# FabricioArendTorres/FlowConductor

Hardware: AMD Instinct MI355X
Metric: log_prob samples/sec, 32xRQ-NSF coupling D=64 K=8 (higher is better)
Workload: dtype f32

## Files before the change

flowconductor_amd/csrc/fc_rq_eval_plan.h:

```cpp
#pragma once
#include <hip/hip_runtime.h>
#include <utility>

#ifndef FC_GEN_SHIFT
#define FC_GEN_SHIFT 0
#endif

namespace fc {

template <class F, int... I>
__device__ __forceinline__ void static_for(F&& f, std::integer_sequence<int, I...>) {
  (f(std::integral_constant<int, I>{}), ...);
}

template <int K, int HOOKS, bool kHookReads, bool kBox>
struct EvalPlan {
  enum Section {
    sInside, sBoxErr, sMaxInit, sRead, sDer,
    sMax, sSub, sExp, sSumInit, sSum, sTot, sRcpX, sRcpY, sKnot, sSelect, sBin, sDelta, sTheta,
    sSoftExp, sSoftFix, sSoftLog, sSoftDer,
    sSoftExp1, sSoftFix1, sSoftLog1, sSoftDer1,
    sDsum, sQuadratic, sT1mt, sDn1, sDnum, sLog, sLval, sYs, sOut, kSections
  };
  struct Sec { int count, weight; };
  static constexpr Sec kSecs[kSections] = {
      {1, 3},
      {kBox ? 1 : 0, 1},
      {1, 1},
      {K, 3},
      {kBox ? K + 1 : K - 1, 1},
      {1, 0},
      {K, 1},
      {K, 4},
      {1, 0},
      {K - 2, 1},
      {1, 1},
      {1, 5},
      {1, 6},
      {2 * (K - 1), 2},
      {1, 3}, {1, 2},
      {1, 5}, {1, 4},
      {1, 6}, {1, 3}, {1, 10}, {1, 3},
      {1, 6}, {1, 3}, {1, 10}, {1, 3},
      {1, 3}, {1, 2},
      {1, 4}, {1, 5}, {1, 4},
      {1, 3}, {1, 1},
      {1, 8}, {1, 3},
  };
  static constexpr int first(int section) {
    int c = 0;
    for (int s = 0; s < section; ++s) c += kSecs[s].count;
    return c;
  }
  static constexpr int kChunks = first(kSections);
  static constexpr int weight(int chunk) {
    int s = 0;
    while (chunk >= kSecs[s].count) chunk -= kSecs[s++].count;
    return kSecs[s].weight;
  }
  static constexpr int hooks_until(int chunk) {
    if (chunk == kChunks - 1) return HOOKS;
    const int start = kHookReads ? 0 : first(sMax);
    int total = 0, acc = 0, hook = 0;
    for (int c = start; c < kChunks; ++c) total += weight(c);
    for (int c = start; c <= chunk; ++c) {
      acc += weight(c);
      while (hook < HOOKS && acc * HOOKS * 100 >= ((hook + 1) * 100 - (FC_GEN_SHIFT)) * total) ++hook;
    }
    return hook;
  }
};

}
```

flowconductor_amd/csrc/fc_rq_eval_straight.inc:

```
{
  using std::integral_constant, std::make_integer_sequence;
  auto chunk_end = [&](auto C) {
    constexpr int c = decltype(C)::value, h0 = c > 0 ? Plan::hooks_until(c - 1) : 0, h1 = Plan::hooks_until(c);
    static_for([&](auto J) { hook(integral_constant<int, h0 + decltype(J)::value>{}); }, make_integer_sequence<int, h1 - h0>{});
  };
#define FC_CHUNK_END(section, i) chunk_end(integral_constant<int, Plan::first(Plan::section) + (i)>{})
  constexpr int H = K / 2;

  const bool inside = (x >= q.left) && (x <= q.right);
  const float xc = inside ? x : q.left;
  FC_CHUNK_END(sInside, 0);
  if constexpr (!kTails) {
    if (!inside) err |= kErrOutsideDomain;
    FC_CHUNK_END(sBoxErr, 0);
  }
  float mx = -INFINITY, my = -INFINITY;
  FC_CHUNK_END(sMaxInit, 0);
  FC_F2 t[K];
  static_for([&](auto I) {
    t[I] = FC_F2{FC_WH(I), FC_WH(K + I)};
    mx = fmaxf(mx, t[I].x);
    my = fmaxf(my, t[I].y);
    FC_CHUNK_END(sRead, I);
  }, make_integer_sequence<int, K>{});
  static_for([&](auto J) {
    FC_DER_ST(kTails ? J + 1 : J, FC_UD(J));
    FC_CHUNK_END(sDer, J);
  }, make_integer_sequence<int, kTails ? K - 1 : K + 1>{});
  const FC_F2 m = {mx, my};
  FC_CHUNK_END(sMax, 0);
  static_for([&](auto I) {
    t[I] = t[I] - m;
    FC_CHUNK_END(sSub, I);
  }, make_integer_sequence<int, K>{});
  static_for([&](auto I) {
    t[I] = FC_F2{__builtin_amdgcn_exp2f(t[I].x), __builtin_amdgcn_exp2f(t[I].y)};
    FC_CHUNK_END(sExp, I);
  }, make_integer_sequence<int, K>{});
  FC_F2 l[H], r[K - 1];
  l[0] = t[0];
  r[K - 2] = t[K - 1];
  FC_CHUNK_END(sSumInit, 0);
  static_for([&](auto N) {
    if constexpr (N < H - 1) {
      l[N + 1] = l[N] + t[N + 1];
      FC_CHUNK_END(sSum, 2 * N);
    }
    r[K - 3 - N] = r[K - 2 - N] + t[K - 2 - N];
    FC_CHUNK_END(sSum, N < H - 1 ? 2 * N + 1 : 2 * N);
  }, make_integer_sequence<int, K - H - 1>{});
  const FC_F2 tot = l[H - 1] + r[H - 1];
  FC_CHUNK_END(sTot, 0);
  const float rsx = div_lean(1.f, tot.x);
  FC_CHUNK_END(sRcpX, 0);
  const float rsy = div_lean(1.f, tot.y);
  const FC_F2 gk = sc1 * FC_F2{rsx, rsy};
  int idx = 0;
  FC_CHUNK_END(sRcpY, 0);
  static_for([&](auto I) {
    FC_F2 next;
    if constexpr (I < H) next = __builtin_elementwise_fma(l[I], gk, kc[I]);
    else next = __builtin_elementwise_fma(r[I], -gk, kc[I]);
    FC_KNOT_ST(I + 1, next);
    FC_CHUNK_END(sKnot, 2 * I);
    FC_COUNT_GE(idx, xc, kInv ? next.y : next.x);
    FC_CHUNK_END(sKnot, 2 * I + 1);
  }, make_integer_sequence<int, K - 1>{});
  const int bin = idx;
  const FC_F2 sel_lo = FC_KNOT_LD(bin, 0), sel_hi = FC_KNOT_LD(bin, 1);
  const float u[2] = {FC_DER_LD(bin, 0), FC_DER_LD(bin, 1)};
  FC_CHUNK_END(sSelect, 0);
  const float xk = sel_lo.x, yk = sel_lo.y;
  const float wk = sel_hi.x - sel_lo.x, hk = sel_hi.y - sel_lo.y;
  FC_CHUNK_END(sBin, 0);
  const float rwk = __builtin_amdgcn_rcpf(wk);
  const float dq = hk * rwk;
  const float delta = __builtin_fmaf(__builtin_fmaf(-wk, dq, hk), rwk, dq);
  FC_CHUNK_END(sDelta, 0);
  float theta;
  if constexpr (!kInv) {
    const float tq = (xc - xk) * rwk;
    theta = __builtin_fmaf(__builtin_fmaf(-wk, tq, xc - xk), rwk, tq);
  }
  FC_CHUNK_END(sTheta, 0);
  float d[2];
  static_for([&](auto N) {
    const float xb = u[N];
    const float xm = fminf(xb, 20.f);
    const float ex = __builtin_amdgcn_exp2f(xm * 1.4426950408889634f);
    FC_CHUNK_END(sSoftExp + 4 * N, 0);
    const float up = 1.f + ex;
    const float rr = ex - (up - 1.f);
    FC_CHUNK_END(sSoftFix + 4 * N, 0);
    const float l1p = __builtin_fmaf(__builtin_amdgcn_logf(up), 0.6931471805599453f, rr * __builtin_amdgcn_rcpf(up));
    FC_CHUNK_END(sSoftLog + 4 * N, 0);
    d[N] = q.min_d + (xb > 20.f ? xb : l1p) * inv_beta;
    FC_CHUNK_END(sSoftDer + 4 * N, 0);
  }, make_integer_sequence<int, 2>{});
  const float d0 = d[0], d1 = d[1];
  const float dsum = d0 + d1 - 2.f * delta;
  FC_CHUNK_END(sDsum, 0);
  if constexpr (kInv) {
    const float rr = xc - yk;
    const float qa = rr * dsum + hk * (delta - d0);
    const float qb = hk * d0 - rr * dsum;
    const float qc = -delta * rr;
    const float disc = qb * qb - 4.f * qa * qc;
    if (inside && !(disc >= 0.f)) err |= kErrDiscriminant;
    theta = div_lean(2.f * qc, -qb - sqrt_lean(disc));
  }
  FC_CHUNK_END(sQuadratic, 0);
  const float t1mt = theta * (1.f - theta);
  const float den = delta + dsum * t1mt;
  FC_CHUNK_END(sT1mt, 0);
  const float omt = 1.f - theta;
  const float dn1 = d1 * (theta * theta) + 2.f * delta * t1mt;
  FC_CHUNK_END(sDn1, 0);
  const float dnum = (delta * delta) * (dn1 + d0 * (omt * omt));
  FC_CHUNK_END(sDnum, 0);
  const float l2v = __builtin_fmaf(-2.f, __builtin_amdgcn_logf(den), __builtin_amdgcn_logf(dnum));
  FC_CHUNK_END(sLog, 0);
  const float lval = l2v * 0.6931471805599453f;
  FC_CHUNK_END(sLval, 0);
  float ys;
  if constexpr (!kInv) {
    const float num = hk * (delta * (theta * theta) + d0 * t1mt);
    ys = yk + div_lean(num, den);
  } else {
    ys = theta * wk + xk;
  }
  FC_CHUNK_END(sYs, 0);
  y = inside ? ys : x;
  lad = inside ? (kInv ? -lval : lval) : 0.f;
  FC_CHUNK_END(sOut, 0);
  static_assert(Plan::kSecs[Plan::sBoxErr].count == (kTails ? 0 : 1) && Plan::kSecs[Plan::sRead].count == K &&
                    Plan::kSecs[Plan::sDer].count == (kTails ? K - 1 : K + 1) && Plan::kSecs[Plan::sSub].count == K &&
                    Plan::kSecs[Plan::sExp].count == K && Plan::kSecs[Plan::sSum].count == (H - 1) + (K - H - 1) &&
                    Plan::kSecs[Plan::sKnot].count == 2 * (K - 1),
                "the plan and this fragment count the same chunks");
#undef FC_CHUNK_END
}
```

flowconductor_amd/csrc/fc_rq_fused3.hip:

```cpp
#include <hip/hip_runtime.h>
#include <stdint.h>
#include <type_traits>
#include "fc_tile.h"
#include "fc_math.h"
#include "fc_rq_op.h"
#include "fc_rq_eval_plan.h"
#include "fc_rq_fused.h"
#include "fc_split.h"
#include "fc_lane.h"
#include "../../include/flowcon_hip.h"

#ifndef FC_ABL
#define FC_ABL 0
#endif

namespace fc {

#ifndef FC_HOOK_MASK
#define FC_HOOK_MASK 0
#endif
#define FC_F2 f2
#ifndef FC_PRIO_PERIOD
#define FC_PRIO_PERIOD 36
#endif

constexpr int kCt3 = 6;
constexpr int kHB = kH + 16;
constexpr int kKnotFloats = (kK + 1) * 64 * 2;
constexpr int kDerFloats = (kK + 1) * 64;
constexpr int kTabBytes = 8 * (kKnotFloats + kDerFloats) * 4;

template <int R>
struct Fused3Lds {
  static constexpr int kHPiece = R * kHB;
  static constexpr int kHbufBytes = 2 * 2 * kHPiece * 2;
  static constexpr int kLpartBytes = 3 * 8 * R * 4;
  static constexpr int kHscaleBytes = 3 * R * 4;
  static constexpr size_t bytes(int d) {
    return (size_t)kHbufBytes + kLpartBytes + kHscaleBytes + kTabBytes + 3 * R * (d + 4) * 4 + kDt * 4;
  }
};

size_t fused3_lds_bytes(int d, int rows) { return rows == 64 ? Fused3Lds<64>::bytes(d) : Fused3Lds<32>::bytes(d); }

template <bool kInv, int R, int XV, bool kFull, bool kPadX>
__global__ __launch_bounds__(512) void rq_fused_linear_kernel3(RQOp<kK> op, FusedArgs a) {
  using L = Fused3Lds<R>;
  constexpr int kHPiece = L::kHPiece;
  constexpr int NB = R / 16;
  constexpr int HV = R / 32;
  extern __shared__ __attribute__((aligned(16))) unsigned char smem3[];
  _Float16* hbuf = reinterpret_cast<_Float16*>(smem3);
  float* lpart = reinterpret_cast<float*>(smem3 + L::kHbufBytes);
  float* hscale = lpart + 3 * 8 * R;
  float* tabs = hscale + 3 * R;
  float* xbuf = tabs + kTabBytes / 4;
  const int D = a.D, XS = kPadX ? D + 4 : D;
  int* cs = reinterpret_cast<int*>(xbuf + 3 * R * (D + 4));

  const int tid = threadIdx.x, wave = tid >> 6, lane = tid & 63;
  const int s16 = lane & 15, g = lane >> 4;
  const int64_t stride = gridDim.x;
  const int64_t tile0 = blockIdx.x;
  if (tile0 >= a.tiles) return;
  if (tid < kDt) cs[tid] = tid < a.dt ? a.cols[tid] : 0;
  const int WD = kFull ? 8 : (a.dt + 3) >> 2;
  const bool dim_ok = kFull || 4 * wave + g < a.dt;
  const bool active = kFull || wave < WD;
  const float inv_div = op.inv_div;
#if FC_ABL & 16
  const uint64_t stamp_r_entry = __builtin_amdgcn_s_memrealtime();
#endif

  constexpr auto slot_param = [](int s) { return s < 16 ? ((s & 1) ? 8 + (s >> 1) : (s >> 1)) : s; };
  f16x8 wh[kCt3][2], wl[kCt3][2];
  float w_unscale;
  {
    float wv[kCt3][2][8];
    float wmax = 0.f;
#pragma unroll
    for (int t = 0; t < kCt3; ++t) {
      const int wdim = 4 * (active ? wave : 0) + (s16 >> 2), wprm = slot_param(4 * t + (s16 & 3));
      const bool wreal = wprm < kPP - 1 && wdim < a.dt;
      const int row = wreal ? wdim * a.wrows + wprm : 0;
      const float wmask = wreal ? 1.f : 0.f;
#pragma unroll
      for (int ks = 0; ks < 2; ++ks) {
        const float4* src = reinterpret_cast<const float4*>(a.wpad + (int64_t)row * kH + 32 * ks + 8 * g);
        const float4 v0 = src[0], v1 = src[1];
        const float v[8] = {v0.x * wmask, v0.y * wmask, v0.z * wmask, v0.w * wmask,
                            v1.x * wmask, v1.y * wmask, v1.z * wmask, v1.w * wmask};
#pragma unroll
        for (int j = 0; j < 8; ++j) {
          wv[t][ks][j] = v[j];
          wmax = fmaxf(wmax, fabsf(v[j]));
        }
      }
    }
#pragma unroll
    for (int o = 32; o > 0; o >>= 1) wmax = fmaxf(wmax, __shfl_xor(wmax, o));
    float w_scale;
    pow2_scale(wmax, w_scale, w_unscale);
#pragma unroll
    for (int t = 0; t < kCt3; ++t)
#pragma unroll
      for (int ks = 0; ks < 2; ++ks)
#pragma unroll
        for (int j = 0; j < 8; ++j) {
          _Float16 ph, pl;
          split2(wv[t][ks][j] * w_scale, ph, pl);
          wh[t][ks][j] = ph;
          wl[t][ks][j] = pl;
        }
  }
  const float wh_mul = (float)((double)inv_div * 1.4426950408889634);
  f32x4 bw[kCt3];
#pragma unroll
  for (int t = 0; t < kCt3; ++t) {
    const int bdim = 4 * (active ? wave : 0) + g;
    const float* bsrc = a.bias + bdim * a.wrows;
    const float m = t < 4 ? wh_mul : op.q.beta;
    const bool bdim_ok = bdim < a.dt;
    auto bias_of = [&](int slot) {
      const int prm = slot_param(slot);
      const bool real = prm < kPP - 1 && bdim_ok;
      return (real ? bsrc[prm] : a.bias[0]) * (real ? m : 0.f);
    };
    bw[t] = f32x4{bias_of(4 * t), bias_of(4 * t + 1), bias_of(4 * t + 2), bias_of(4 * t + 3)};
  }
  const double span_x = (double)op.q.right - (double)op.q.left, span_y = (double)op.q.top - (double)op.q.bottom;
  const f2 sc1 = {(float)(span_x * (double)op.q.cw), (float)(span_y * (double)op.q.ch)};
  auto knot_const = [&](int i) {
    if (i < kK / 2)
      return f2{(float)((double)op.q.left + span_x * (double)op.q.min_w * (double)(i + 1)),
                (float)((double)op.q.bottom + span_y * (double)op.q.min_h * (double)(i + 1))};
    return f2{(float)((double)op.q.right - span_x * (double)op.q.min_w * (double)(kK - 1 - i)),
              (float)((double)op.q.top - span_y * (double)op.q.min_h * (double)(kK - 1 - i))};
  };
  f2 kc[kK - 1];
  static_for([&](auto I) { kc[I] = knot_const(I); }, std::make_integer_sequence<int, kK - 1>{});

  float* ktab = tabs + wave * (kKnotFloats + kDerFloats) + lane * 2;
  float* dtab = tabs + wave * (kKnotFloats + kDerFloats) + kKnotFloats + lane;
  *reinterpret_cast<f2*>(ktab) = f2{op.q.left, op.q.bottom};
  *reinterpret_cast<f2*>(ktab + kK * 128) = f2{op.q.right, op.q.top};
  dtab[0] = op.q.tail_const * op.q.beta;
  dtab[kK * 64] = op.q.tail_const * op.q.beta;

  uint32_t err = 0;
  int mycol = 0;
  const int xvec = R * D / 4;
  constexpr bool kCarry = kFull && XV <= 2;
  float4 hv0, hv1, xv0, xv1, xv2, xv3;
  hv0 = hv1 = xv0 = xv1 = xv2 = xv3 = float4{0.f, 0.f, 0.f, 0.f};
  int64_t fetched = tile0;
  auto fetch = [&](int64_t t) __attribute__((always_inline)) {
    fetched = t;
    if (FC_ABL & 8) t = tile0;
    const float4* hg = reinterpret_cast<const float4*>(a.h + t * R * kH);
    hv0 = hg[tid];
    if constexpr (HV > 1 && kFull) hv1 = hg[tid + 512];
    const float4* xg = reinterpret_cast<const float4*>(a.x + t * R * D);
    xv0 = xg[tid < xvec ? tid : 0];
    if constexpr (kCarry) {
      if constexpr (XV > 1) xv1 = xg[tid + 512 < xvec ? tid + 512 : 0];
      if constexpr (XV > 2) xv2 = xg[tid + 1024 < xvec ? tid + 1024 : 0];
      if constexpr (XV > 3) xv3 = xg[tid + 1536 < xvec ? tid + 1536 : 0];
    }
  };
  auto xslot = [&](int buf, int i) __attribute__((always_inline)) {
    if constexpr (!kPadX) return reinterpret_cast<float4*>(xbuf + buf * R * XS + 4 * i);
    const int e = i * 4, r = e / D, c = e - r * D;
    return reinterpret_cast<float4*>(xbuf + (buf * R + r) * XS + c);
  };
  auto park_h = [&](int buf, int xbuf3, int k, const float4& hvk) __attribute__((always_inline)) {
    const int c = (tid & 15) * 4, r = (tid >> 4) + 32 * k;
#if FC_ABL & 32
    {
      _Float16* dst = hbuf + (buf * 2 * R + r) * kHB + c;
      *reinterpret_cast<u32x2*>(dst) = u32x2{__float_as_uint(hvk.x) & 0x3bff3bffu, __float_as_uint(hvk.y) & 0x3bff3bffu};
      *reinterpret_cast<u32x2*>(dst + kHPiece) = u32x2{__float_as_uint(hvk.z) & 0x3bff3bffu, __float_as_uint(hvk.w) & 0x3bff3bffu};
      if ((tid & 15) == 0) hscale[xbuf3 * R + r] = 1.f;
      return;
    }
#endif
    const float v[4] = {hvk.x, hvk.y, hvk.z, hvk.w};
    const float m = row16_allmax(fmaxf(fmaxf(fabsf(v[0]), fabsf(v[1])), fmaxf(fabsf(v[2]), fabsf(v[3]))));
    float sc, un;
    pow2_scale(m, sc, un);
    u32x2 p0, p1;
#pragma unroll
    for (int j = 0; j < 2; ++j) {
      uint32_t ph, pl;
      split2_pair(v[2 * j], v[2 * j + 1], sc, ph, pl);
      p0[j] = ph; p1[j] = pl;
    }
    _Float16* dst = hbuf + (buf * 2 * R + r) * kHB + c;
    *reinterpret_cast<u32x2*>(dst) = p0;
    *reinterpret_cast<u32x2*>(dst + kHPiece) = p1;
    if ((tid & 15) == 0) hscale[xbuf3 * R + r] = un;
  };
  auto park = [&](int hb2, int x3) __attribute__((always_inline)) {
    park_h(hb2, x3, 0, hv0);
    if constexpr (HV > 1 && !kFull)
      hv1 = reinterpret_cast<const float4*>(a.h + ((FC_ABL & 8) ? tile0 : fetched) * R * kH)[tid + 512];
    if constexpr (HV > 1) park_h(hb2, x3, 1, hv1);
    if (tid < xvec) *xslot(x3, tid) = xv0;
    if constexpr (!kCarry && XV > 1) {
      const float4* xg = reinterpret_cast<const float4*>(a.x + ((FC_ABL & 8) ? tile0 : fetched) * R * D);
      xv1 = xg[tid + 512 < xvec ? tid + 512 : 0];
      if constexpr (XV > 2) xv2 = xg[tid + 1024 < xvec ? tid + 1024 : 0];
      if constexpr (XV > 3) xv3 = xg[tid + 1536 < xvec ? tid + 1536 : 0];
    }
    if constexpr (XV > 1) if (tid + 512 < xvec) *xslot(x3, tid + 512) = xv1;
    if constexpr (XV > 2) if (tid + 1024 < xvec) *xslot(x3, tid + 1024) = xv2;
    if constexpr (XV > 3) if (tid + 1536 < xvec) *xslot(x3, tid + 1536) = xv3;
  };
  auto hfrag = [&](int hb, int blk, int hp, int ks) {
    return *reinterpret_cast<const f16x8*>(hbuf + ((hb * 2 + hp) * R + 16 * blk + s16) * kHB + 32 * ks + 8 * g);
  };

  auto mfma_n = [&](auto N, f32x4 (&acc)[kCt3], const f16x8& bcur) {
    constexpr int n = decltype(N)::value, term = n / 12, ks = (n / 6) % 2, t = n % 6;
    const f16x8& aop = term == 0 ? wl[t][ks] : wh[t][ks];
    acc[t] = __builtin_amdgcn_mfma_f32_16x16x32_f16(aop, bcur, n < kCt3 ? f32x4{0.f, 0.f, 0.f, 0.f} : acc[t], 0, 0, 0);
  };
  constexpr auto term_h = [](int term) { return term == 1 ? 1 : 0; };

#define FC_ALL36(M)                                                                                          \
  M(0) M(1) M(2) M(3) M(4) M(5) M(6) M(7) M(8) M(9) M(10) M(11) M(12) M(13) M(14) M(15) M(16) M(17) M(18)     \
  M(19) M(20) M(21) M(22) M(23) M(24) M(25) M(26) M(27) M(28) M(29) M(30) M(31) M(32) M(33) M(34) M(35)

  auto produce_only = [&](f32x4 (&acc)[kCt3], int hb, int blk) {
    f16x8 bcur = hfrag(hb, blk, term_h(0), 0);
    auto one = [&](auto N) {
      constexpr int n = decltype(N)::value;
      if constexpr (n % 6 == 0 && n > 0) bcur = hfrag(hb, blk, term_h(n / 12), (n / 6) % 2);
      mfma_n(N, acc, bcur);
    };
#define FC_S(n) one(std::integral_constant<int, n>{});
    FC_ALL36(FC_S)
#undef FC_S
  };

  auto step = [&](const f32x4 (&pa)[kCt3], int xb, int cblk, f32x4 (&acc)[kCt3], int hb, int pblk, float& lad_out) {
    float* xr = xbuf + (xb * R + 16 * cblk + s16) * XS + mycol;
    const float x = *xr;
    const float c_d = hscale[xb * R + 16 * cblk + s16] * w_unscale;
    const float c_wh = c_d * wh_mul;
    const float c_ud = c_d * op.q.beta;
    f16x8 bcur, bnext = hfrag(hb, pblk, term_h(0), 0);
    auto hook = [&](auto N) {
      constexpr int n = decltype(N)::value;
      if constexpr (n % 6 == 0) {
        bcur = bnext;
        if constexpr (n + 6 < 36) bnext = hfrag(hb, pblk, term_h((n + 6) / 12), ((n + 6) / 6) % 2);
      }
      if constexpr (!(FC_ABL & 4)) mfma_n(N, acc, bcur);
      if constexpr (n % (FC_PRIO_PERIOD / 4) == FC_PRIO_PERIOD / 4 - 1)
        __builtin_amdgcn_s_setprio(3 - ((n + 1) % FC_PRIO_PERIOD) / (FC_PRIO_PERIOD / 4));
      __builtin_amdgcn_sched_barrier(FC_HOOK_MASK);
    };
    constexpr int K = kK;
    constexpr bool kTails = true;
    using Plan = EvalPlan<kK, 6 * kCt3, true, false>;
    const RQParams& q = op.q;
    const float inv_beta = op.inv_beta;
    float y, lad;
    __builtin_amdgcn_s_setprio(3);
    __builtin_amdgcn_sched_barrier(0);
#define FC_HOOK(n) hook(std::integral_constant<int, n>{});
#define FC_WH_SLOT(i) ((i) < 8 ? 2 * (i) : 2 * ((i) - 8) + 1)
#define FC_WH(i) __builtin_fmaf(pa[FC_WH_SLOT(i) >> 2][FC_WH_SLOT(i) & 3], c_wh, bw[FC_WH_SLOT(i) >> 2][FC_WH_SLOT(i) & 3])
#define FC_UD(j) __builtin_fmaf(pa[((j) + 16) >> 2][((j) + 16) & 3], c_ud, bw[((j) + 16) >> 2][((j) + 16) & 3])
#define FC_KNOT_ST(slot, v) *reinterpret_cast<f2*>(ktab + (slot) * 128) = (v)
#define FC_KNOT_LD(i, off) *reinterpret_cast<const f2*>(ktab + ((i) + (off)) * 128)
#define FC_DER_ST(slot, v) dtab[(slot) * 64] = (v)
#define FC_DER_LD(i, off) dtab[((i) + (off)) * 64]
#define FC_COUNT_GE(count, a, b)                                                              \
  do {                                                                                        \
    const float fc_b_ = (b);                                                                  \
    asm("v_cmp_ge_f32 vcc, %1, %2\n\tv_addc_co_u32 %0, vcc, 0, %0, vcc" : "+v"(count) : "v"(a), "v"(fc_b_) : "vcc"); \
  } while (0)
#if FC_ABL & 1
    FC_ALL36(FC_HOOK)
    y = x + (FC_WH(0) + FC_WH(5) + FC_WH(10) + FC_WH(15) + FC_UD(0) + FC_UD(5)) * 0.f + q.left * 0.f;
    lad = 0.f;
#else
#include "fc_rq_eval_straight.inc"
#endif
#undef FC_COUNT_GE
#undef FC_DER_LD
#undef FC_DER_ST
#undef FC_KNOT_LD
#undef FC_KNOT_ST
#undef FC_UD
#undef FC_WH
#undef FC_WH_SLOT
#undef FC_HOOK
    if (dim_ok) *xr = y;
    lad_out = dim_ok ? lad : 0.f;
  };
  auto after_steps = [&](int xb, const float (&lb)[NB]) __attribute__((always_inline)) {
    if constexpr (NB == 4) {
      const float l = lane_merge16(lb[0], lane_merge32(lb[2], lb[3]));
      lpart[(xb * 8 + wave) * R + 16 * rows4_sum4_index(g) + s16] = l;
    } else {
      const float m = lane_merge32(lb[0], lb[1]);
      const float l = m + lane_xor16(m, lane);
      if ((g & 1) == 0) lpart[(xb * 8 + wave) * R + 16 * (g >> 1) + s16] = l;
    }
  };

#if FC_ABL & 16
  const uint64_t stamp_c0 = __builtin_amdgcn_s_memtime(), stamp_r0 = __builtin_amdgcn_s_memrealtime();
#endif
#if FC_ABL & 16
  uint64_t barrier_wait = 0, phase_cyc[6] = {0, 0, 0, 0, 0, 0}, phase_t = __builtin_amdgcn_s_memtime();
#define FC_PHASE(k)                                              \
  do {                                                           \
    const uint64_t now = __builtin_amdgcn_s_memtime();           \
    phase_cyc[k] += now - phase_t;                               \
    phase_t = now;                                               \
  } while (0)
#define FC_TIMED_BARRIER()                                        \
  do {                                                            \
    const uint64_t b0 = __builtin_amdgcn_s_memtime();             \
    __syncthreads();                                              \
    barrier_wait += __builtin_amdgcn_s_memtime() - b0;            \
  } while (0)
#else
#define FC_TIMED_BARRIER() __syncthreads()
#define FC_PHASE(k)
#endif
  f32x4 acc0[kCt3], acc1[kCt3];
#pragma unroll
  for (int t = 0; t < kCt3; ++t) acc0[t] = acc1[t] = f32x4{0.f, 0.f, 0.f, 0.f};
  auto write_out = [&](int64_t t, int x3) __attribute__((always_inline)) {
    float4* yg = reinterpret_cast<float4*>(a.y + t * R * D);
#pragma unroll
    for (int k = 0; k < XV; ++k)
      if (tid + 512 * k < xvec) yg[tid + 512 * k] = *xslot(x3, tid + 512 * k);
    if (tid < R) {
      const float* lp = lpart + x3 * 8 * R + tid;
      float l = lp[0];
#pragma unroll
      for (int w = 1; w < 8; ++w)
        if (w < WD) l += lp[w * R];
      a.logabsdet[t * R + tid] = a.accumulate ? a.logabsdet[t * R + tid] + l : l;
    }
  };
  fetch(tile0);
  park(0, 0);
  __syncthreads();
  mycol = cs[(4 * wave + g) & (kDt - 1)];
  if (active) produce_only(acc0, 0, 0);
  int hb = 0, x3 = 0;
  int64_t prev_tile = -1;
  for (int64_t tile = tile0; tile < a.tiles; tile += stride) {
    const bool has_next = tile + stride < a.tiles;
    const int x3n = x3 == 2 ? 0 : x3 + 1, x3p = x3 == 0 ? 2 : x3 - 1;
    FC_PHASE(0);
    if (has_next) fetch(tile + stride);
    float lb[NB];
#pragma unroll
    for (int b = 0; b < NB; ++b) lb[b] = 0.f;
    if (active) {
      step(acc0, x3, 0, acc1, hb, 1, lb[0]);
      if constexpr (NB == 4) {
        step(acc1, x3, 1, acc0, hb, 2, lb[1]);
        lb[0] = lane_merge32(lb[0], lb[1]);
        step(acc0, x3, 2, acc1, hb, 3, lb[2]);
      }
    }
    FC_PHASE(1);
    if (has_next) park(hb ^ 1, x3n);
    FC_PHASE(2);
    FC_TIMED_BARRIER();
    FC_PHASE(3);
    if (prev_tile >= 0) write_out(prev_tile, x3p);
    FC_PHASE(5);
    if (active) {
      step(acc1, x3, NB - 1, acc0, hb ^ 1, 0, lb[NB - 1]);
      after_steps(x3, lb);
    }
    FC_PHASE(4);
    prev_tile = tile;
    hb ^= 1;
    x3 = x3n;
  }
  __syncthreads();
  if (prev_tile >= 0) write_out(prev_tile, x3 == 0 ? 2 : x3 - 1);
#if FC_ABL & 16
  if (tid == 0) {
    a.y[tile0 * R * D] = (float)(__builtin_amdgcn_s_memtime() - stamp_c0);
    a.y[tile0 * R * D + 1] = (float)(__builtin_amdgcn_s_memrealtime() - stamp_r0);
    a.y[tile0 * R * D + 2] = (float)(stamp_r0 - stamp_r_entry);
    a.y[tile0 * R * D + 3] = (float)(stamp_r_entry & 0xffffff);
  }
  if (lane == 0) {
    a.y[tile0 * R * D + 4 + wave] = (float)barrier_wait;
#pragma unroll
    for (int k = 0; k < 6; ++k) a.y[tile0 * R * D + 12 + wave * 6 + k] = (float)phase_cyc[k];
  }
#endif
  if (err && a.err) atomicOr(a.err, err);
}
#undef FC_ALL36
#undef FC_TIMED_BARRIER
#undef FC_PHASE

template <bool kInv, int R, int XV, bool kFull, bool kPadX>
static hipError_t launch_cfg(const RQOp<kK>& op, const FusedArgs& a, unsigned grid, hipStream_t stream) {
  const size_t lds = Fused3Lds<R>::bytes(a.D);
  if (lds > 160 * 1024) return hipErrorInvalidConfiguration;
  static PerDeviceOnce attr;
  const hipError_t ea = ensure_max_dynamic_lds(
      attr, reinterpret_cast<const void*>(&rq_fused_linear_kernel3<kInv, R, XV, kFull, kPadX>), 160 * 1024);
  if (ea != hipSuccess) return ea;
  hipLaunchKernelGGL((rq_fused_linear_kernel3<kInv, R, XV, kFull, kPadX>), dim3(grid), dim3(512), lds, stream, op, a);
  return hipGetLastError();
}

template <bool kInv, int R, int XV>
static hipError_t launch_one(const RQOp<kK>& op, const FusedArgs& a, unsigned grid, hipStream_t stream) {
  if (a.D & 3) return launch_cfg<kInv, R, XV, false, false>(op, a, grid, stream);
  return a.dt == kDt ? launch_cfg<kInv, R, XV, true, true>(op, a, grid, stream)
                     : launch_cfg<kInv, R, XV, false, true>(op, a, grid, stream);
}

hipError_t launch_fused3(const RQOp<kK>& op, const FusedArgs& a, int rows, unsigned grid, hipStream_t stream) {
  const bool inv = op.q.inverse != 0;
  if (rows == 64) {
    if (a.D <= 32) return inv ? launch_one<true, 64, 1>(op, a, grid, stream) : launch_one<false, 64, 1>(op, a, grid, stream);
    if (a.D <= 64) return inv ? launch_one<true, 64, 2>(op, a, grid, stream) : launch_one<false, 64, 2>(op, a, grid, stream);
    return inv ? launch_one<true, 64, 4>(op, a, grid, stream) : launch_one<false, 64, 4>(op, a, grid, stream);
  }
  if (a.D <= 64) return inv ? launch_one<true, 32, 1>(op, a, grid, stream) : launch_one<false, 32, 1>(op, a, grid, stream);
  return inv ? launch_one<true, 32, 2>(op, a, grid, stream) : launch_one<false, 32, 2>(op, a, grid, stream);
}

}
```

flowconductor_amd/csrc/fc_rq_fused4_body.h:

```cpp
#include <hip/hip_runtime.h>
#include <stdint.h>
#include <type_traits>
#include <utility>
#include "fc_device.h"
#include "fc_lane.h"
#include "fc_math.h"
#include "fc_rq_eval_plan.h"
#include "fc_rq_fused_general.h"
#include "fc_rq_op.h"
#include "fc_split.h"
#include "fc_tile.h"

#define FC_F4_CAT2(a, b) a##b
#define FC_F4_CAT(a, b) FC_F4_CAT2(a, b)

namespace fc {
namespace FC_F4_CAT(f4, FC_F4_NAME) {

#define FC_F2 f2
constexpr int K = FC_F4_K;
constexpr bool kTails = FC_F4_TAILS != 0;
constexpr int P = kTails ? 3 * K - 1 : 3 * K + 1;
constexpr int CT = (P + 3) / 4;
constexpr int PP = 4 * CT;
constexpr int NM = 6 * CT;
using Plan = EvalPlan<K, NM, false, !kTails>;
constexpr int R = 32;
constexpr int kHB = 64 + 16;
constexpr int kBiasRow = 36;
constexpr int kKnotFloats = (K + 1) * 64 * 2;
constexpr int kDerFloats = (K + 1) * 64;
constexpr int kTabBytes = 8 * (kKnotFloats + kDerFloats) * 4;
constexpr int kHPiece = R * kHB;
constexpr int kHbufBytes = 2 * 2 * kHPiece * 2;
constexpr int kLpartBytes = 3 * 8 * R * 4;
constexpr int kHscaleBytes = 3 * R * 4;
constexpr int kBiasBytes = 8 * 4 * kBiasRow * 4;
static_assert(PP <= 32 && K <= 11 && K >= 4, "accumulator slots / knot constants");

constexpr size_t lds_bytes(int d) {
  return (size_t)kHbufBytes + kLpartBytes + kHscaleBytes + kTabBytes + kBiasBytes + (size_t)3 * R * (d + 4) * 4 + 32 * 4;
}

template <bool kInv, int XV, bool kFull, bool kPadX>
__global__ __launch_bounds__(512) void rq_fused_linear_kernel4(RQOp<K> op, GenArgs a) {
  extern __shared__ __attribute__((aligned(16))) unsigned char smem4[];
  _Float16* hbuf = reinterpret_cast<_Float16*>(smem4);
  float* lpart = reinterpret_cast<float*>(smem4 + kHbufBytes);
  float* hscale = lpart + 3 * 8 * R;
  float* tabs = hscale + 3 * R;
  float* bias_lds = tabs + kTabBytes / 4;
  float* xbuf = bias_lds + 8 * 4 * kBiasRow;
  const int D = a.D, XS = kPadX ? D + 4 : D;
  int* cs = reinterpret_cast<int*>(xbuf + 3 * R * (D + 4));

  const int tid = threadIdx.x, wave = tid >> 6, lane = tid & 63;
  const int s16 = lane & 15, g = lane >> 4;
  const int64_t stride = gridDim.x;
  const int64_t tile0 = blockIdx.x;
  if (tile0 >= a.tiles) return;
  if (tid < 32) cs[tid] = a.cols[tid < a.dt ? tid : 0];
  const int WD = kFull ? 8 : (a.dt + 3) >> 2;
  const bool dim_ok = kFull || 4 * wave + g < a.dt;
  const bool active = kFull || wave < WD;
  const int grp = active ? wave : 0;

  auto slot_param = [](int s) { return s < 2 * K ? ((s & 1) ? K + (s >> 1) : (s >> 1)) : s; };
  f16x8 wh[CT][2], wl[CT][2];
  {
    const f16x8* wbase = a.wfrag + (size_t)grp * 2 * CT * 2 * 64;
#pragma unroll
    for (int t = 0; t < CT; ++t) {
      const int p = slot_param(4 * t + (lane & 3));
      const int st = p >> 2, sl = (lane & ~3) | (p & 3);
#pragma unroll
      for (int ks = 0; ks < 2; ++ks) {
        wh[t][ks] = wbase[((ks * CT + st) * 2 + 0) * 64 + sl];
        wl[t][ks] = wbase[((ks * CT + st) * 2 + 1) * 64 + sl];
      }
    }
  }
  const float w_unscale = a.wun[grp];
  const float inv_div = op.inv_div;
  const float wh_mul = (float)((double)inv_div * 1.4426950408889634);
  for (int i = tid; i < WD * 4 * PP; i += 512) {
    const int row = i / PP, slot = i - row * PP;
    const int prm = slot_param(slot);
    bias_lds[row * kBiasRow + slot] = a.bias[row * PP + prm] * (slot < 2 * K ? wh_mul : op.q.beta);
  }
  const f32x4* bwp = reinterpret_cast<const f32x4*>(bias_lds + (grp * 4 + g) * kBiasRow);

  const RQParams& q = op.q;
  const f2 sc1 = {q.sc1x, q.sc1y};
  f2 kc[K - 1];
  static_for([&](auto I) { kc[I] = f2{q.kcx[I], q.kcy[I]}; }, std::make_integer_sequence<int, K - 1>{});

  float* ktab = tabs + wave * (kKnotFloats + kDerFloats) + lane * 2;
  float* dtab = tabs + wave * (kKnotFloats + kDerFloats) + kKnotFloats + lane;
  *reinterpret_cast<f2*>(ktab) = f2{q.left, q.bottom};
  *reinterpret_cast<f2*>(ktab + K * 128) = f2{q.right, q.top};
  if constexpr (kTails) {
    dtab[0] = q.tail_const * q.beta;
    dtab[K * 64] = q.tail_const * q.beta;
  }

  uint32_t err = 0;
  int mycol = 0;
  const int xvec = R * D / 4;
  float4 hv0, xv0, xv1;
  hv0 = xv0 = xv1 = float4{0.f, 0.f, 0.f, 0.f};
  auto fetch = [&](int64_t t) __attribute__((always_inline)) {
    hv0 = reinterpret_cast<const float4*>(a.h + t * R * 64)[tid];
    const float4* xg = reinterpret_cast<const float4*>(a.x + t * R * D);
    xv0 = xg[tid < xvec ? tid : 0];
    if constexpr (XV > 1) xv1 = xg[tid + 512 < xvec ? tid + 512 : 0];
  };
  auto xslot = [&](int buf, int i) __attribute__((always_inline)) {
    if constexpr (!kPadX) return reinterpret_cast<float4*>(xbuf + buf * R * XS + 4 * i);
    const int e = i * 4, r = e / D, c = e - r * D;
    return reinterpret_cast<float4*>(xbuf + (buf * R + r) * XS + c);
  };
  auto park = [&](int hb2, int x3) __attribute__((always_inline)) {
    const int c = (tid & 15) * 4, r = tid >> 4;
    const float v[4] = {hv0.x, hv0.y, hv0.z, hv0.w};
    const float m = row16_allmax(fmaxf(fmaxf(fabsf(v[0]), fabsf(v[1])), fmaxf(fabsf(v[2]), fabsf(v[3]))));
    float sc, un;
    pow2_scale(m, sc, un);
    u32x2 p0, p1;
#pragma unroll
    for (int j = 0; j < 2; ++j) {
      uint32_t ph, pl;
      split2_pair(v[2 * j], v[2 * j + 1], sc, ph, pl);
      p0[j] = ph; p1[j] = pl;
    }
    _Float16* dst = hbuf + (hb2 * 2 * R + r) * kHB + c;
    *reinterpret_cast<u32x2*>(dst) = p0;
    *reinterpret_cast<u32x2*>(dst + kHPiece) = p1;
    if ((tid & 15) == 0) hscale[x3 * R + r] = un;
    if (tid < xvec) *xslot(x3, tid) = xv0;
    if constexpr (XV > 1) if (tid + 512 < xvec) *xslot(x3, tid + 512) = xv1;
  };
  auto hfrag = [&](int hb, int blk, int hp, int ks) {
    return *reinterpret_cast<const f16x8*>(hbuf + ((hb * 2 + hp) * R + 16 * blk + s16) * kHB + 32 * ks + 8 * g);
  };
  auto mfma_n = [&](auto N, f32x4 (&acc)[CT], const f16x8& bcur) {
    constexpr int n = decltype(N)::value, term = n / (2 * CT), ks = (n / CT) % 2, t = n % CT;
    const f16x8& aop = term == 0 ? wl[t][ks] : wh[t][ks];
    acc[t] = __builtin_amdgcn_mfma_f32_16x16x32_f16(aop, bcur, n < CT ? f32x4{0.f, 0.f, 0.f, 0.f} : acc[t], 0, 0, 0);
  };
  constexpr auto term_h = [](int term) { return term == 1 ? 1 : 0; };

  auto produce_only = [&](f32x4 (&acc)[CT], int hb, int blk) {
    f16x8 bcur = hfrag(hb, blk, term_h(0), 0);
    static_for([&](auto N) {
      constexpr int n = decltype(N)::value;
      if constexpr (n % CT == 0 && n > 0) bcur = hfrag(hb, blk, term_h(n / (2 * CT)), (n / CT) % 2);
      mfma_n(N, acc, bcur);
    }, std::make_integer_sequence<int, NM>{});
  };

  auto step = [&](f32x4 (&acc)[CT], int xb, int cblk, int hb, int pblk, float& lad_out) {
    float* xr = xbuf + (xb * R + 16 * cblk + s16) * XS + mycol;
    const float x = *xr;
    const float c_d = hscale[xb * R + 16 * cblk + s16] * w_unscale;
    const float c_wh = c_d * wh_mul;
    const float c_ud = c_d * q.beta;
    f32x4 bw[CT];
#pragma unroll
    for (int t = 0; t < CT; ++t) bw[t] = bwp[t];
    f16x8 bcur, bnext = hfrag(hb, pblk, term_h(0), 0);
    constexpr int PQ = (NM + 3) / 4;
    auto hook = [&](auto N) {
      constexpr int n = decltype(N)::value;
      if constexpr (n % CT == 0) {
        bcur = bnext;
        if constexpr (n + CT < NM) bnext = hfrag(hb, pblk, term_h((n + CT) / (2 * CT)), ((n + CT) / CT) % 2);
      }
      mfma_n(N, acc, bcur);
      if constexpr (n % PQ == PQ - 1 || n == NM - 1) __builtin_amdgcn_s_setprio(3 - ((n + 1) % NM) / PQ);
      __builtin_amdgcn_sched_barrier(0);
    };
    const float inv_beta = op.inv_beta;
    float y, lad;
    __builtin_amdgcn_s_setprio(3);
    __builtin_amdgcn_sched_barrier(0);
#define FC_WH_SLOT(i) ((i) < K ? 2 * (i) : 2 * ((i) - K) + 1)
#define FC_WH(i) __builtin_fmaf(acc[FC_WH_SLOT(i) >> 2][FC_WH_SLOT(i) & 3], c_wh, bw[FC_WH_SLOT(i) >> 2][FC_WH_SLOT(i) & 3])
#define FC_UD(j) __builtin_fmaf(acc[((j) + 2 * K) >> 2][((j) + 2 * K) & 3], c_ud, bw[((j) + 2 * K) >> 2][((j) + 2 * K) & 3])
#define FC_KNOT_ST(slot, v) *reinterpret_cast<f2*>(ktab + (slot) * 128) = (v)
#define FC_KNOT_LD(i, off) *reinterpret_cast<const f2*>(ktab + ((i) + (off)) * 128)
#define FC_DER_ST(slot, v) dtab[(slot) * 64] = (v)
#define FC_DER_LD(i, off) dtab[((i) + (off)) * 64]
#define FC_COUNT_GE(count, a, b)                                                              \
  do {                                                                                        \
    const float fc_b_ = (b);                                                                  \
    asm("v_cmp_ge_f32 vcc, %1, %2\n\tv_addc_co_u32 %0, vcc, 0, %0, vcc" : "+v"(count) : "v"(a), "v"(fc_b_) : "vcc"); \
  } while (0)
#include "fc_rq_eval_straight.inc"
#undef FC_COUNT_GE
#undef FC_DER_LD
#undef FC_DER_ST
#undef FC_KNOT_LD
#undef FC_KNOT_ST
#undef FC_UD
#undef FC_WH
#undef FC_WH_SLOT
    if (dim_ok) *xr = y;
    lad_out = dim_ok ? lad : 0.f;
  };
  auto after_steps = [&](int xb, float l0, float l1) __attribute__((always_inline)) {
    const float m = lane_merge32(l0, l1);
    const float l = m + lane_xor16(m, lane);
    if ((g & 1) == 0) lpart[(xb * 8 + wave) * R + 16 * (g >> 1) + s16] = l;
  };

  f32x4 acc[CT];
#pragma unroll
  for (int t = 0; t < CT; ++t) acc[t] = f32x4{0.f, 0.f, 0.f, 0.f};
  auto write_out = [&](int64_t t, int x3) __attribute__((always_inline)) {
    float4* yg = reinterpret_cast<float4*>(a.y + t * R * D);
#pragma unroll
    for (int k = 0; k < XV; ++k)
      if (tid + 512 * k < xvec) yg[tid + 512 * k] = *xslot(x3, tid + 512 * k);
    if (tid < R) {
      const float* lp = lpart + x3 * 8 * R + tid;
      float l = lp[0];
#pragma unroll
      for (int w = 1; w < 8; ++w)
        if (w < WD) l += lp[w * R];
      a.logabsdet[t * R + tid] = a.accumulate ? a.logabsdet[t * R + tid] + l : l;
    }
  };
#ifdef FC_F4_STAMP
  const uint64_t stamp_c0 = __builtin_amdgcn_s_memtime(), stamp_r0 = __builtin_amdgcn_s_memrealtime();
  uint64_t phase_cyc[6] = {0, 0, 0, 0, 0, 0}, phase_t = stamp_c0;
#define FC_PHASE(k)                                              \
  do {                                                           \
    const uint64_t now = __builtin_amdgcn_s_memtime();           \
    phase_cyc[k] += now - phase_t;                               \
    phase_t = now;                                               \
  } while (0)
#else
#define FC_PHASE(k)
#endif
  fetch(tile0);
  park(0, 0);
  __syncthreads();
  mycol = cs[(4 * wave + g) & 31];
  if (active) produce_only(acc, 0, 0);
  int hb = 0, x3 = 0;
  int64_t prev_tile = -1;
  for (int64_t tile = tile0; tile < a.tiles; tile += stride) {
    const bool has_next = tile + stride < a.tiles;
    const int x3n = x3 == 2 ? 0 : x3 + 1, x3p = x3 == 0 ? 2 : x3 - 1;
    FC_PHASE(0);
    if (has_next) fetch(tile + stride);
    float lb0 = 0.f, lb1 = 0.f;
    if (active) step(acc, x3, 0, hb, 1, lb0);
    FC_PHASE(1);
    if (has_next) park(hb ^ 1, x3n);
    FC_PHASE(2);
    __syncthreads();
    FC_PHASE(3);
    if (prev_tile >= 0) write_out(prev_tile, x3p);
    FC_PHASE(4);
    if (active) {
      step(acc, x3, 1, hb ^ 1, 0, lb1);
      after_steps(x3, lb0, lb1);
    }
    FC_PHASE(5);
    prev_tile = tile;
    hb ^= 1;
    x3 = x3n;
  }
  __syncthreads();
  if (prev_tile >= 0) write_out(prev_tile, x3 == 0 ? 2 : x3 - 1);
#ifdef FC_F4_STAMP
  if (tid == 0) {
    a.y[tile0 * R * D] = (float)(__builtin_amdgcn_s_memtime() - stamp_c0);
    a.y[tile0 * R * D + 1] = (float)(__builtin_amdgcn_s_memrealtime() - stamp_r0);
  }
  if (lane == 0) {
#pragma unroll
    for (int k = 0; k < 6; ++k) a.y[tile0 * R * D + 4 + wave * 6 + k] = (float)phase_cyc[k];
  }
#endif
#undef FC_PHASE
  if (err && a.err) atomicOr(a.err, err);
}

template <bool kInv, int XV, bool kFull, bool kPadX>
static hipError_t launch_cfg(const RQOp<K>& op, const GenArgs& a, hipStream_t stream) {
  const size_t lds = lds_bytes(a.D);
  if (lds > 160 * 1024) return hipErrorInvalidConfiguration;
  static PerDeviceOnce attr;
  const hipError_t ea = ensure_max_dynamic_lds(
      attr, reinterpret_cast<const void*>(&rq_fused_linear_kernel4<kInv, XV, kFull, kPadX>), 160 * 1024);
  if (ea != hipSuccess) return ea;
  const int64_t cus = device_cu_count();
  const unsigned grid = (unsigned)(cus < a.tiles ? cus : a.tiles);
  hipLaunchKernelGGL((rq_fused_linear_kernel4<kInv, XV, kFull, kPadX>), dim3(grid), dim3(512), lds, stream, op, a);
  return hipGetLastError();
}

template <bool kInv, int XV>
static hipError_t launch_one(const RQOp<K>& op, const GenArgs& a, hipStream_t stream) {
  if (a.D & 3) return launch_cfg<kInv, XV, false, false>(op, a, stream);
  return a.dt == 32 ? launch_cfg<kInv, XV, true, true>(op, a, stream) : launch_cfg<kInv, XV, false, true>(op, a, stream);
}

}

hipError_t FC_F4_CAT(launch_fused4_, FC_F4_NAME)(const RQParams& q, const GenArgs& a, hipStream_t stream) {
  using namespace FC_F4_CAT(f4, FC_F4_NAME);
  RQOp<K> op;
  op.q = q;
  op.inv_div = 1.f / q.wh_div;
  op.inv_beta = 1.f / q.beta;
  const bool inv = q.inverse != 0;
  if (R * a.D / 4 <= 512) return inv ? launch_one<true, 1>(op, a, stream) : launch_one<false, 1>(op, a, stream);
  return inv ? launch_one<true, 2>(op, a, stream) : launch_one<false, 2>(op, a, stream);
}
size_t FC_F4_CAT(fused4_lds_bytes_, FC_F4_NAME)(int d) { return FC_F4_CAT(f4, FC_F4_NAME)::lds_bytes(d); }

}
```

Before: 56.64 million.

## Interleave softplus transcendentals with bin math and rebalance MFMA hook schedule

Restructures the rational-quadratic spline tail so both softplus exp/log/rcp evaluations are issued together and interleaved with the bin delta/theta computation. This shortens the dependent chain and packs the transcendental latencies together. It replaces div_lean and sqrt_lean with explicit rcp plus Newton refinement, and adds an inverse-path section split. The eval plan gains per-section shadow weights, including a configurable select shadow, to redistribute interleaved MFMA hooks. Changed weights shift MFMA placement and could unbalance the overlap, and the refined-sqrt edge handling could differ slightly numerically.

```diff
diff --git a/flowconductor_amd/csrc/fc_rq_eval_plan.h b/flowconductor_amd/csrc/fc_rq_eval_plan.h
--- a/flowconductor_amd/csrc/fc_rq_eval_plan.h
+++ b/flowconductor_amd/csrc/fc_rq_eval_plan.h
@@ -5,7 +5,6 @@
 #ifndef FC_GEN_SHIFT
 #define FC_GEN_SHIFT 0
 #endif
-
 namespace fc {
 
 template <class F, int... I>
@@ -13,39 +12,49 @@
   (f(std::integral_constant<int, I>{}), ...);
 }
 
-template <int K, int HOOKS, bool kHookReads, bool kBox>
+template <int K, int HOOKS, bool kHookReads, bool kBox, bool kInv, int kSelectShadow = 0>
 struct EvalPlan {
   enum Section {
     sInside, sBoxErr, sMaxInit, sRead, sDer,
-    sMax, sSub, sExp, sSumInit, sSum, sTot, sRcpX, sRcpY, sKnot, sSelect, sBin, sDelta, sTheta,
-    sSoftExp, sSoftFix, sSoftLog, sSoftDer,
-    sSoftExp1, sSoftFix1, sSoftLog1, sSoftDer1,
-    sDsum, sQuadratic, sT1mt, sDn1, sDnum, sLog, sLval, sYs, sOut, kSections
+    sMax, sSub, sExp, sSumInit, sSum, sTot, sRcpX, sRcpY, sKnot, sSelect,
+    sBin, sTrans1, sShadow1, sTrans2, sShadow2, sL1p, sSoftDer, sBinOnly, sDsum,
+    sQuadratic, sRoot, sThetaInv, sTailInv,
+    sDen, sLog, sLval, sYs, sOut, kSections
   };
-  struct Sec { int count, weight; };
+  struct Sec { int count, weight, shadow; };
   static constexpr Sec kSecs[kSections] = {
-      {1, 3},
-      {kBox ? 1 : 0, 1},
-      {1, 1},
-      {K, 3},
-      {kBox ? K + 1 : K - 1, 1},
-      {1, 0},
-      {K, 1},
-      {K, 4},
-      {1, 0},
-      {K - 2, 1},
-      {1, 1},
-      {1, 5},
-      {1, 6},
-      {2 * (K - 1), 2},
-      {1, 3}, {1, 2},
-      {1, 5}, {1, 4},
-      {1, 6}, {1, 3}, {1, 10}, {1, 3},
-      {1, 6}, {1, 3}, {1, 10}, {1, 3},
-      {1, 3}, {1, 2},
-      {1, 4}, {1, 5}, {1, 4},
-      {1, 3}, {1, 1},
-      {1, 8}, {1, 3},
+      {1, 3, 0},
+      {kBox ? 1 : 0, 1, 0},
+      {1, 1, 0},
+      {K, 3, 0},
+      {kBox ? K + 1 : K - 1, 1, 0},
+      {1, 0, 0},
+      {K, 1, 0},
+      {K, 4, 0},
+      {1, 0, 0},
+      {K - 2, 1, 0},
+      {1, 1, 0},
+      {1, 5, 0},
+      {1, 6, 0},
+      {2 * (K - 1), 2, 0},
+      {1, 3, kSelectShadow},
+      {1, 9, 0},
+      {1, 6, 0},
+      {1, 4, 0},
+      {1, 8, 0},
+      {1, 8, 0},
+      {1, 4, 0},
+      {1, 8, 0},
+      {1, 8, 0},
+      {1, 2, 0},
+      {kInv ? 1 : 0, 12, 0},
+      {kInv ? 1 : 0, 10, 0},
+      {kInv ? 1 : 0, 3, 0},
+      {kInv ? 1 : 0, 7, 0},
+      {1, 10, 0},
+      {1, 6, 0}, {1, 2, 0},
+      {kInv ? 0 : 1, 4, 0},
+      {1, 3, 0},
   };
   static constexpr int first(int section) {
     int c = 0;
@@ -56,7 +65,7 @@
   static constexpr int weight(int chunk) {
     int s = 0;
     while (chunk >= kSecs[s].count) chunk -= kSecs[s++].count;
-    return kSecs[s].weight;
+    return kSecs[s].weight + kSecs[s].shadow;
   }
   static constexpr int hooks_until(int chunk) {
     if (chunk == kChunks - 1) return HOOKS;
diff --git a/flowconductor_amd/csrc/fc_rq_eval_straight.inc b/flowconductor_amd/csrc/fc_rq_eval_straight.inc
--- a/flowconductor_amd/csrc/fc_rq_eval_straight.inc
+++ b/flowconductor_amd/csrc/fc_rq_eval_straight.inc
@@ -72,64 +72,90 @@
   FC_CHUNK_END(sSelect, 0);
   const float xk = sel_lo.x, yk = sel_lo.y;
   const float wk = sel_hi.x - sel_lo.x, hk = sel_hi.y - sel_lo.y;
+  const float dx = xc - (kInv ? yk : xk);
+  const float xb0 = u[0], xb1 = u[1];
+  const float xs0 = fminf(xb0, 20.f) * 1.4426950408889634f, xs1 = fminf(xb1, 20.f) * 1.4426950408889634f;
   FC_CHUNK_END(sBin, 0);
   const float rwk = __builtin_amdgcn_rcpf(wk);
+  const float ex0 = __builtin_amdgcn_exp2f(xs0), ex1 = __builtin_amdgcn_exp2f(xs1);
+  FC_CHUNK_END(sTrans1, 0);
   const float dq = hk * rwk;
+  float tq;
+  if constexpr (!kInv) tq = dx * rwk;
+  const float up0 = 1.f + ex0, up1 = 1.f + ex1;
+  FC_CHUNK_END(sShadow1, 0);
+  const float lg0 = __builtin_amdgcn_logf(up0), lg1 = __builtin_amdgcn_logf(up1);
+  const float ru0 = __builtin_amdgcn_rcpf(up0), ru1 = __builtin_amdgcn_rcpf(up1);
+  FC_CHUNK_END(sTrans2, 0);
   const float delta = __builtin_fmaf(__builtin_fmaf(-wk, dq, hk), rwk, dq);
-  FC_CHUNK_END(sDelta, 0);
   float theta;
+  if constexpr (!kInv) theta = __builtin_fmaf(__builtin_fmaf(-wk, tq, dx), rwk, tq);
+  const float rr0 = ex0 - (up0 - 1.f), rr1 = ex1 - (up1 - 1.f);
+  FC_CHUNK_END(sShadow2, 0);
+  const float l1p0 = __builtin_fmaf(lg0, 0.6931471805599453f, rr0 * ru0);
+  const float l1p1 = __builtin_fmaf(lg1, 0.6931471805599453f, rr1 * ru1);
+  FC_CHUNK_END(sL1p, 0);
+  const float d0 = q.min_d + (xb0 > 20.f ? xb0 : l1p0) * inv_beta;
+  const float d1 = q.min_d + (xb1 > 20.f ? xb1 : l1p1) * inv_beta;
+  FC_CHUNK_END(sSoftDer, 0);
+  const float de2 = delta * delta, twod = 2.f * delta;
+  float omt, t1mt, th2, om2, tdt, dth2, qc;
   if constexpr (!kInv) {
-    const float tq = (xc - xk) * rwk;
-    theta = __builtin_fmaf(__builtin_fmaf(-wk, tq, xc - xk), rwk, tq);
+    omt = 1.f - theta;
+    t1mt = theta * omt;
+    th2 = theta * theta;
+    om2 = omt * omt;
+    tdt = twod * t1mt;
+    dth2 = delta * th2;
+  } else {
+    qc = -delta * dx;
   }
-  FC_CHUNK_END(sTheta, 0);
-  float d[2];
-  static_for([&](auto N) {
-    const float xb = u[N];
-    const float xm = fminf(xb, 20.f);
-    const float ex = __builtin_amdgcn_exp2f(xm * 1.4426950408889634f);
-    FC_CHUNK_END(sSoftExp + 4 * N, 0);
-    const float up = 1.f + ex;
-    const float rr = ex - (up - 1.f);
-    FC_CHUNK_END(sSoftFix + 4 * N, 0);
-    const float l1p = __builtin_fmaf(__builtin_amdgcn_logf(up), 0.6931471805599453f, rr * __builtin_amdgcn_rcpf(up));
-    FC_CHUNK_END(sSoftLog + 4 * N, 0);
-    d[N] = q.min_d + (xb > 20.f ? xb : l1p) * inv_beta;
-    FC_CHUNK_END(sSoftDer + 4 * N, 0);
-  }, make_integer_sequence<int, 2>{});
-  const float d0 = d[0], d1 = d[1];
-  const float dsum = d0 + d1 - 2.f * delta;
+  FC_CHUNK_END(sBinOnly, 0);
+  const float dsum = d0 + d1 - twod;
   FC_CHUNK_END(sDsum, 0);
   if constexpr (kInv) {
-    const float rr = xc - yk;
-    const float qa = rr * dsum + hk * (delta - d0);
-    const float qb = hk * d0 - rr * dsum;
-    const float qc = -delta * rr;
+    const float rds = dx * dsum;
+    const float qa = rds + hk * (delta - d0);
+    const float qb = hk * d0 - rds;
     const float disc = qb * qb - 4.f * qa * qc;
     if (inside && !(disc >= 0.f)) err |= kErrDiscriminant;
-    theta = div_lean(2.f * qc, -qb - sqrt_lean(disc));
+    FC_CHUNK_END(sQuadratic, 0);
+    const float sr = __builtin_amdgcn_sqrtf(disc);
+    const float qn = 2.f * qc;
+    const float hrs = 0.5f * __builtin_amdgcn_rcpf(sr);
+    const float sq = !(sr > 0.f) ? sr : __builtin_fmaf(__builtin_fmaf(-sr, sr, disc), hrs, sr);
+    const float qd = -qb - sq;
+    const float rqd = __builtin_amdgcn_rcpf(qd);
+    FC_CHUNK_END(sRoot, 0);
+    const float qq = qn * rqd;
+    theta = __builtin_fmaf(__builtin_fmaf(-qd, qq, qn), rqd, qq);
+    FC_CHUNK_END(sThetaInv, 0);
+    omt = 1.f - theta;
+    t1mt = theta * omt;
+    th2 = theta * theta;
+    om2 = omt * omt;
+    tdt = twod * t1mt;
+    FC_CHUNK_END(sTailInv, 0);
   }
-  FC_CHUNK_END(sQuadratic, 0);
-  const float t1mt = theta * (1.f - theta);
   const float den = delta + dsum * t1mt;
-  FC_CHUNK_END(sT1mt, 0);
-  const float omt = 1.f - theta;
-  const float dn1 = d1 * (theta * theta) + 2.f * delta * t1mt;
-  FC_CHUNK_END(sDn1, 0);
-  const float dnum = (delta * delta) * (dn1 + d0 * (omt * omt));
-  FC_CHUNK_END(sDnum, 0);
-  const float l2v = __builtin_fmaf(-2.f, __builtin_amdgcn_logf(den), __builtin_amdgcn_logf(dnum));
+  const float dnum = de2 * ((d1 * th2 + tdt) + d0 * om2);
+  float num;
+  if constexpr (!kInv) num = hk * (dth2 + d0 * t1mt);
+  FC_CHUNK_END(sDen, 0);
+  const float lden = __builtin_amdgcn_logf(den), ldnum = __builtin_amdgcn_logf(dnum);
+  float rden;
+  if constexpr (!kInv) rden = __builtin_amdgcn_rcpf(den);
   FC_CHUNK_END(sLog, 0);
-  const float lval = l2v * 0.6931471805599453f;
+  const float lval = __builtin_fmaf(-2.f, lden, ldnum) * 0.6931471805599453f;
   FC_CHUNK_END(sLval, 0);
   float ys;
   if constexpr (!kInv) {
-    const float num = hk * (delta * (theta * theta) + d0 * t1mt);
-    ys = yk + div_lean(num, den);
+    const float yq = num * rden;
+    ys = yk + __builtin_fmaf(__builtin_fmaf(-den, yq, num), rden, yq);
+    FC_CHUNK_END(sYs, 0);
   } else {
     ys = theta * wk + xk;
   }
-  FC_CHUNK_END(sYs, 0);
   y = inside ? ys : x;
   lad = inside ? (kInv ? -lval : lval) : 0.f;
   FC_CHUNK_END(sOut, 0);
diff --git a/flowconductor_amd/csrc/fc_rq_fused3.hip b/flowconductor_amd/csrc/fc_rq_fused3.hip
--- a/flowconductor_amd/csrc/fc_rq_fused3.hip
+++ b/flowconductor_amd/csrc/fc_rq_fused3.hip
@@ -22,6 +22,10 @@
 #define FC_F2 f2
 #ifndef FC_PRIO_PERIOD
 #define FC_PRIO_PERIOD 36
+#endif
+
+#ifndef FC_SHADOW_SELECT
+#define FC_SHADOW_SELECT 16
 #endif
 
 constexpr int kCt3 = 6;
@@ -263,7 +267,7 @@
     };
     constexpr int K = kK;
     constexpr bool kTails = true;
-    using Plan = EvalPlan<kK, 6 * kCt3, true, false>;
+    using Plan = EvalPlan<kK, 6 * kCt3, true, false, kInv, kFull ? FC_SHADOW_SELECT : 0>;
     const RQParams& q = op.q;
     const float inv_beta = op.inv_beta;
     float y, lad;
diff --git a/flowconductor_amd/csrc/fc_rq_fused4_body.h b/flowconductor_amd/csrc/fc_rq_fused4_body.h
--- a/flowconductor_amd/csrc/fc_rq_fused4_body.h
+++ b/flowconductor_amd/csrc/fc_rq_fused4_body.h
@@ -24,7 +24,8 @@
 constexpr int CT = (P + 3) / 4;
 constexpr int PP = 4 * CT;
 constexpr int NM = 6 * CT;
-using Plan = EvalPlan<K, NM, false, !kTails>;
+template <bool kInv>
+using PlanOf = EvalPlan<K, NM, false, !kTails, kInv>;
 constexpr int R = 32;
 constexpr int kHB = 64 + 16;
 constexpr int kBiasRow = 36;
@@ -181,6 +182,7 @@
       __builtin_amdgcn_sched_barrier(0);
     };
     const float inv_beta = op.inv_beta;
+    using Plan = PlanOf<kInv>;
     float y, lad;
     __builtin_amdgcn_s_setprio(3);
     __builtin_amdgcn_sched_barrier(0);
```

Result: no change. 57.18 million (median of 6 runs) (+0.9%).
